# saugns/saugns

Measured on AMD Instinct MI355X. Metric: mono samples/sec/GPU @ N voices (depth-3 FM), higher is better.
Workload: dtype f32 (f64 table interpolation, u32 phase)

## Files before the change

### saugns_amd/csrc/hip_backend.hip

```cpp
#include <hip/hip_runtime.h>
#include "hip_backend.h"
#include "launch_plan.h"
#include "sau_dev_ops.h"
#include <stdio.h>
#include <stdlib.h>
#include <string.h>
#include <deque>
#include <map>
#include <memory>
#include <mutex>
#include <string>
#include <type_traits>
#include <vector>

namespace sauhip {

using namespace saudev;
using sauengine::BackendConfig;
using sauengine::tune_env;
using sauengine::SegmentDesc;
using namespace sauplan;

#include "k_common.h"
#include "k_block_loop.h"
// ... 127 lines not shown
		err = std::string(pinned ? "hipHostMalloc: " : "hipMalloc: ") + hipGetErrorString(e);
		return nullptr;
	}
	return q;
}
static void pool_free(bool pinned, void *q, size_t bytes) {
	if (!q) return;
	if (!BufPool::get().give(pinned, q, bytes)) { if (pinned) (void)hipHostFree(q); else (void)hipFree(q); }
}

static std::mutex &attr_mutex() { static std::mutex *m = new std::mutex; return *m; }
static bool raise_lds_attr(const void *fn, size_t lds, int dev, std::string &err) {
	static std::map<std::pair<const void *, int>, size_t> *slots = new std::map<std::pair<const void *, int>, size_t>;
	std::lock_guard<std::mutex> lk(attr_mutex());
	size_t &configured = (*slots)[std::make_pair(fn, dev & 15)];
	if (lds > configured) {
		hipError_t e = hipFuncSetAttribute(fn, hipFuncAttributeMaxDynamicSharedMemorySize, (int)lds);
		if (e != hipSuccess) { err = std::string("hipFuncSetAttribute: ") + hipGetErrorString(e); return false; }
		configured = lds;
	}
	return true;
}

enum : unsigned { FK_WIDE = 1, FK_TAIL = 2, FK_CUB = 4, FK_INNER = 8, FK_LANEMAJOR = 16 };
static const void *fast_kernel_fn(int build, uint32_t rows, unsigned form) {
	struct Entry { int build; uint32_t rows; unsigned form; const void *fn; };
#define FK(build, form, ...) {build, FK_ROWS(__VA_ARGS__), form, (const void *)fast_kernel<__VA_ARGS__>}
#define FK_ROWS(rows, ...) rows
	static const Entry table[] = {
		FK(0, 0, 2, 0), FK(0, 0, 4, 0), FK(0, 0, 5, 0), FK(0, 0, 6, 0), FK(0, 0, 8, 0),
		FK(1, 0, 2, 1), FK(1, 0, 4, 1),
		FK(2, 0, 2, 2), FK(2, 0, 4, 2), FK(2, 0, 5, 2), FK(2, 0, 6, 2), FK(2, 0, 8, 2),
		FK(3, 0, 4, 3), FK(3, 0, 5, 3), FK(3, 0, 6, 3),
		FK(0, FK_WIDE, 6, 0, false, true), FK(0, FK_WIDE, 8, 0, false, true), FK(0, FK_WIDE, 10, 0, false, true), FK(0, FK_WIDE, 12, 0, false, true),
		FK(2, FK_WIDE | FK_TAIL, 8, 2, false, true, true), FK(2, FK_WIDE, 8, 2, false, true), FK(2, FK_TAIL, 8, 2, false, false, true),
		FK(2, FK_CUB, (int)FAST_CUB_ROWS, 2, true),
		FK(0, FK_WIDE | FK_INNER | FK_LANEMAJOR, 12, 0, false, true, false, true, true), FK(0, FK_WIDE | FK_INNER, 12, 0, false, true, false, true),
		FK(0, FK_CUB, (int)FAST_CUB_ROWS, 0, true)};
#undef FK
#undef FK_ROWS
	for (const Entry &e : table)
		if (e.build == build && e.rows == rows && e.form == form) return e.fn;
	return nullptr;
}
static const void *repair_kernel_fn(uint32_t rows, bool wide) {
	if (wide)
		return rows == 12 ? (const void *)repair_kernel<12, true> : rows == 10 ? (const void *)repair_kernel<10, true>
		     : rows == 8 ? (const void *)repair_kernel<8, true> : rows == 6 ? (const void *)repair_kernel<6, true> : nullptr;
	return rows == 8 ? (const void *)repair_kernel<8> : rows == 6 ? (const void *)repair_kernel<6> : rows == 5 ? (const void *)repair_kernel<5>
	     : rows == 4 ? (const void *)repair_kernel<4> : rows == 2 ? (const void *)repair_kernel<2> : nullptr;
}
static const void *render_kernel_fn(uint32_t W, uint32_t T, uint32_t V, bool HB) {
	struct Entry { uint32_t W, T, V; bool HB; const void *fn; };
#define RK(W, T, V, HB) {W, T, V, HB, (const void *)render_kernel<W, T, V, HB>}
	static const Entry table[] = {
		RK(1, 4, 8, false), RK(1, 3, 8, false), RK(1, 2, 8, false), RK(1, 1, 8, false),
		RK(1, 4, 16, false), RK(1, 3, 16, false), RK(1, 2, 16, false), RK(1, 1, 16, false),
		RK(1, 1, 1, true), RK(1, 1, 1, false), RK(4, 4, 1, false), RK(8, 2, 1, false)};
#undef RK
	for (const Entry &e : table)
		if (e.W == W && e.T == T && e.V == V && e.HB == HB) return e.fn;
	return nullptr;
}

template <typename T, bool PINNED> struct PoolBuf {
	T *p = nullptr;
	size_t cap = 0, bytes = 0;
// ... 711 lines not shown
		}
		j.early_mixed_blocks = mixed_blocks;
		fp.range_mode = 0; fp.f_lo = 0; fp.f_hi = 0; fp.range_last = 0;
		return true;
	}

	bool launch_closed_form(Job &j, std::string &err) {
		const SegmentDesc &seg = j.seg;
		const FastPlan &k = j.fk;
		FastParams &fp = j.fp;
		fp.dyn_chunks = k.tasks.dyn_chunks; fp.dyn_static = k.tasks.dyn_static; fp.dyn_small = k.tasks.dyn_small;
		if (k.queues) {
			fp.inmix_flags = k.inmix_flags;
			fp.inmix_div_s = k.div.s; fp.inmix_div_m = k.div.m;
			if (k.inmix) {
				fp.inmix_stream = sets_[j.set].mstreams.p;
				fp.inmix_pcm_offset = seg.pcm_offset;
				hipLaunchKernelGGL(premix_kernel, dim3((seg.n_voices + 63) / 64), dim3(64), 0, stream_, fp);
				j.inmix_live = true;
			}
		}
		if (k.inner != INNER_NONE) {
			const bool lm = k.inner == INNER_LANE_MAJOR;
			const void *ik = fast_kernel_fn(0, 12, FK_WIDE | FK_INNER | (lm ? FK_LANEMAJOR : 0u));
			const size_t lds = k.inner_lds();
			FastParams ep = fp;
			ep.mode = 0; ep.edge_only = 1; ep.dyn_static = 1; ep.dyn_chunks = 2; ep.dyn_small = 0; ep.inmix_flags = 0;
			if (!launch_build(j, err, 0, k.rows, k.grid_edge, &ep, false, true)) j.launched = false;
			fp.mode = 0;
			void *iargs[] = {(void *)&fp};
			if (!raise_lds_attr(ik, lds, dev_, err)) return false;
			if (fp.inmix_flags && !pcm_hazard(err)) return false;
			HIP_OK(hipLaunchKernel(ik, dim3(k.grid), dim3(1024), iargs, lds, stream_));
			if (inner_report_) fprintf(stderr, "[sau-amd] inner: %s, %u voices\n", lm ? "lane-major" : "row-major", seg.n_voices);
		} else {
			if (inner_report_) fprintf(stderr, "[sau-amd] inner: none (rows %u, wide %d, chunks %u), %u voices\n", k.rows, k.wide_cf ? 1 : 0, fp.dyn_chunks, seg.n_voices);
			if (fp.inmix_flags && (!rows_hazard(j, err) || !pcm_hazard(err))) return false;
			launch_fast(j, err, 0);
		}
		fp.dyn_chunks = 0; fp.inmix_flags = 0; fp.dyn_small = 0;
		return true;
	}

	bool launch_cub(Job &j, std::string &err) {
		if (!j.fp.cub_ok) return true;
		const FastPlan &k = j.fk;
		FastParams q = k.main_build == 2 ? j.cfp : j.fp;
		q.n_fast = k.n_fast_cf; q.rows = FAST_CUB_ROWS; q.mode = 0; q.only_multi = 0;
		q.dyn_chunks = k.tasks_cub.dyn_chunks; q.dyn_static = k.tasks_cub.dyn_static;
		const size_t qlds = k.launch_lds(0, FAST_CUB_ROWS, false, true);
		const void *ck = fast_kernel_fn(0, FAST_CUB_ROWS, FK_CUB);
		if (!raise_lds_attr(ck, qlds, dev_, err)) return false;
		void *qargs[] = {(void *)&q};
		if (!rows_hazard(j, err)) return false;
		HIP_OK(hipLaunchKernel(ck, dim3(k.grid_cub), dim3(1024), qargs, qlds, stream_));
		return true;
	}
// ... 1393 lines not shown
```

### saugns_amd/csrc/k_fast_group_lm.h

```cpp
		const int j0 = l * T;
		const int t0 = (int)(cg * GF) - (int)H + j0;
		const uint32_t om = ((1u << T) - 1u) & ~((1u << min(max((int)H - j0, 0), T)) - 1u);
		auto prev32 = [&](const uint32_t *x, int k) -> uint32_t { return k > 0 ? x[k - 1] : lane_prev(x[T - 1]); };
		auto prev64 = [&](const double *x, int k) -> double { return k > 0 ? x[k - 1] : lane_prev(x[T - 1]); };
		const bool quads = ((cg * GF - H) & 3u) == 0;
		auto store_row = [&](float *row, const float *x, const bool nt) {
			uint32_t o = om;
			asm volatile("" : "+v"(o));
			if (quads) {
#pragma unroll
				for (int q = 0; q < T / 4; ++q) {
					const uint32_t oq = (o >> (4 * q)) & 15u;
					if (oq == 15u) {
						const fk_f32x4 v4 = {x[4 * q], x[4 * q + 1], x[4 * q + 2], x[4 * q + 3]};
						fk_f32x4 *p = (fk_f32x4 *)(row + t0 + 4 * q);
						if (nt) FK_VSTORE(p, v4); else *p = v4;
					} else if (oq != 0u) {
#pragma unroll
						for (int u = 0; u < 4; ++u)
							if ((oq >> u) & 1u) { if (nt) FK_VSTORE(&row[t0 + 4 * q + u], x[4 * q + u]); else row[t0 + 4 * q + u] = x[4 * q + u]; }
					}
				}
			} else {
#pragma unroll
// ... 32 lines not shown
					bool done = false;
					if (FK_COMMON && f.tab >= 0 && !has_fpm && !(f.ramp & 2)) {
						uint32_t ph[T];
						{
							uint32_t acc = f.phase0 + f.inc * (uint32_t)(t0 + 1);
#pragma unroll
							for (int k = 0; k < T; ++k) { ph[k] = acc; acc += f.inc; }
						}
						bool ok = true;
						if (has_pm) {
							float pm[T];
							bool big = false;
#pragma unroll
							for (int k = 0; k < T; ++k) {
								pm[k] = blk[k];
								big |= !(fabsf(pm[k]) < 0x1p20f);
							}
							ok = !__any(big);
#pragma unroll
							for (int k = 0; k < T; ++k) ph[k] += rint32w_p31_small(pm[k]);
						}
						if (ok) {
							const uint32_t ltab = tabs + (uint32_t)f.tab * FkTab<WIDE>::BYTES;
							double Is[T];
#pragma unroll
							for (int k = 0; k < T; ++k) Is[k] = fk_poly(fk_entry<WIDE>(ltab, ph[k]), ph[k]);
							if (FK_CONSTD && !has_pm && f.inc != 0) {
								const double x = (double)div_f32_normal(f.diff_scale, (float)(int32_t)f.inc);
#pragma unroll
								for (int k = 0; k < T; ++k)
									s[k] = (float)((Is[k] - prev64(Is, k)) * x + (double)f.diff_offset);
								done = true;
							} else {
								uint32_t dmin = 0xffffffffu;
#pragma unroll
								for (int k = 0; k < T; ++k) {
									uint32_t pp = prev32(ph, k);
									if (k == 0) asm("" : "+v"(pp));
									const int32_t d = (int32_t)(ph[k] - pp);
									dmin = min(dmin, (uint32_t)d);
									s[k] = wosc_diff(Is[k], prev64(Is, k), d, f.diff_scale, f.diff_offset);
								}
								done = true;
								if (__any(dmin == 0u)) {
									uint32_t hz = 0;
#pragma unroll
									for (int k = 0; k < T; ++k) hz |= ph[k] == prev32(ph, k) ? 1u << k : 0u;
									done = !__any((hz & dm) != 0u);
								}
							}
						}
					}
					if (!done) {
						uint32_t ph[T];
						double Is[T];
						float fv[T];
						{
							uint32_t acc = f.phase0 + f.inc * (uint32_t)(t0 + 1);
#pragma unroll
							for (int k = 0; k < T; ++k) { ph[k] = acc; acc += f.inc; fv[k] = f.fc; }
						}
						if (has_pm && !has_fpm) {
							float pm[T];
							bool big = false;
#pragma unroll
							for (int k = 0; k < T; ++k) {
								pm[k] = blk[k];
								big |= !(fabsf(pm[k]) < 0x1p20f);
							}
							if (!__any(big)) {
#pragma unroll
								for (int k = 0; k < T; ++k) ph[k] += rint32w_p31_small(pm[k]);
							} else {
#pragma unroll
								for (int k = 0; k < T; ++k) ph[k] += rint32w_p31(pm[k]);
							}
						} else if (has_fpm) {
#pragma unroll
							for (int k = 0; k < T; ++k) ph[k] += pm_offset32(false, true, 0.f, blk[k], fv[k]);
						}
						if (f.tab >= 0) {
							const uint32_t ltab = tabs + (uint32_t)f.tab * FkTab<WIDE>::BYTES;
#pragma unroll
							for (int k = 0; k < T; ++k) Is[k] = fk_poly(fk_entry<WIDE>(ltab, ph[k]), ph[k]);
						} else {
							const uint32_t wave = (f.type >> 8) & 0xff;
							const HerpC23 *g23 = P.g_c23 + (size_t)wave * WAVE_LEN;
							const HerpC01 *g01 = P.g_c01 + (size_t)wave * WAVE_LEN;
#pragma unroll
							for (int k = 0; k < T; ++k) {
								const uint32_t ind = ph[k] >> SLEN_BITS;
								Is[k] = herp_poly(g23[ind], g01[ind], ph[k]);
							}
						}
						uint32_t hz = 0;
						if (FK_CONSTD && !has_pm && !has_fpm && f.inc != 0) {
							const double x = (double)div_f32_normal(f.diff_scale, (float)(int32_t)f.inc);
#pragma unroll
							for (int k = 0; k < T; ++k) {
								const double pIs = prev64(Is, k);
								s[k] = (float)((Is[k] - pIs) * x + (double)f.diff_offset);
							}
						} else {
#pragma unroll
							for (int k = 0; k < T; ++k) {
								const uint32_t pph = prev32(ph, k);
								const double pIs = prev64(Is, k);
// ... 146 lines not shown
```

### saugns_amd/csrc/k_fast_voice.h

```cpp
#ifndef FK_TEMPORAL_ROWS
#define FK_VSTORE(p, v) __builtin_nontemporal_store((v), (p))
#else
#define FK_VSTORE(p, v) (*(p) = (v))
#endif
#ifndef FK_TEMPORAL_ROWS
#define FK_CSTORE(p, v) __builtin_nontemporal_store((v), (p))
#define FK_CLOAD(p) __builtin_nontemporal_load(p)
#else
#define FK_CSTORE(p, v) (*(p) = (v))
#define FK_CLOAD(p) (*(p))
#endif

__device__ __forceinline__ uint32_t lane_prev(uint32_t x) {
	return (uint32_t)__builtin_amdgcn_update_dpp(0, (int)x, 0x138 , 0xf, 0xf, true);
}
__device__ __forceinline__ double lane_prev(double x) {
	const uint32_t lo = lane_prev((uint32_t)__double2loint(x));
	const uint32_t hi = lane_prev((uint32_t)__double2hiint(x));
	return __hiloint2double((int)hi, (int)lo);
}

typedef double __attribute__((ext_vector_type(2))) fk_f64x2;
typedef float __attribute__((ext_vector_type(2))) fk_f32x2;
typedef float __attribute__((ext_vector_type(4))) fk_f32x4;
typedef const fk_f64x2 __attribute__((address_space(3))) *fk_lds_f64x2;
typedef const fk_f32x2 __attribute__((address_space(3))) *fk_lds_f32x2;
struct FkHerp { double c3, c2, c1, c0; };
template <bool WIDE, bool TAB0 = false>
__device__ __forceinline__ FkHerp fk_entry(const uint32_t tab, const uint32_t ph) {
	FkHerp h;
	if (WIDE && TAB0) {
		const uint32_t a = (ph >> (SLEN_BITS - 4)) & ((WAVE_LEN - 1) << 4);
		const fk_f64x2 hi = *(fk_lds_f64x2)(uintptr_t)a;
		const fk_f64x2 lo = *(fk_lds_f64x2)(uintptr_t)(a + FkTab<true>::C01);
		h.c3 = hi.x; h.c2 = hi.y; h.c1 = lo.x; h.c0 = lo.y;
	} else if (WIDE) {
		uint32_t ind = ph >> SLEN_BITS;
		asm("" : "+v"(ind));
		const uint32_t a = tab + (ind << 4);
		const fk_f64x2 hi = *(fk_lds_f64x2)(uintptr_t)a;
		const fk_f64x2 lo = *(fk_lds_f64x2)(uintptr_t)(a + FkTab<true>::C01);
		h.c3 = hi.x; h.c2 = hi.y; h.c1 = lo.x; h.c0 = lo.y;
	} else {
		const uint32_t ind = ph >> SLEN_BITS;
		const fk_f64x2 hi = *(fk_lds_f64x2)(uintptr_t)(tab + ind * 16u);
		const fk_f32x2 lo = *(fk_lds_f32x2)(uintptr_t)(tab + FkTab<false>::C01 + ind * 8u);
		h.c3 = hi.x; h.c2 = hi.y; h.c1 = (double)lo.x; h.c0 = (double)lo.y;
	}
	return h;
}
__device__ __forceinline__ double fk_poly(const FkHerp &h, const uint32_t ph) {
	const double x = (double)(ph & (SLEN - 1));
	return ((h.c3 * x + h.c2) * x + h.c1) * x + h.c0;
}
__device__ __forceinline__ double fk_poly_rise(const FkHerp &h, const uint32_t ph) {
	const double x = (double)(ph & (SLEN - 1));
	return ((h.c3 * x + h.c2) * x + h.c1) * x;
}
template <bool WIDE>
__device__ __forceinline__ void fk_stage_tables(const FastParams &P, unsigned char *lds, const uint32_t tid, const uint32_t nthreads) {
	for (uint32_t t = 0; t < P.n_tabs; ++t) {
		const uint32_t wave = P.wave_of_tab[t];
		const uint4 *s23 = (const uint4 *)(P.g_c23 + (size_t)wave * WAVE_LEN);
		uint4 *d23 = (uint4 *)(lds + (size_t)t * FkTab<WIDE>::BYTES);
		for (uint32_t i = tid; i < WAVE_LEN; i += nthreads) d23[i] = s23[i];
		const HerpC01 *s01 = P.g_c01 + (size_t)wave * WAVE_LEN;
		if (WIDE) {
			fk_f64x2 *d01 = (fk_f64x2 *)(lds + (size_t)t * FkTab<WIDE>::BYTES + FkTab<WIDE>::C01);
			for (uint32_t i = tid; i < WAVE_LEN; i += nthreads) { fk_f64x2 v; v.x = (double)s01[i].c1; v.y = (double)s01[i].c0; d01[i] = v; }
		} else {
			uint2 *d01 = (uint2 *)(lds + (size_t)t * FkTab<WIDE>::BYTES + FkTab<WIDE>::C01);
			for (uint32_t i = tid; i < WAVE_LEN; i += nthreads) d01[i] = ((const uint2 *)s01)[i];
		}
	}
}

__device__ __forceinline__ FastStep load_step_uniform(const FastStep *p) {
	const_u32_ptr q = (const_u32_ptr)(uintptr_t)p;
	union { FastStep s; uint32_t u[20]; } c;
#pragma unroll
	for (int i = 0; i < 20; ++i) c.u[i] = q[i];
	return c.s;
}

template <int T, int SCAN, bool REPAIR = false, bool CUB = false, bool WIDE = false, int SPLIT = 0 , bool TAIL = false>
__device__ __forceinline__ void fast_voice(const FastParams &P, const uint32_t v, const FastInfo &fi,
		float *slots, unsigned long long *carry, const uint32_t tabs , const int l,
		const uint32_t wpv, const uint32_t cstart, unsigned long long *lring = nullptr,
		const uint32_t dyn_c = 0, const uint32_t dyn_k = 0 ,
		const uint32_t vpos = ~0u ,
		const uint32_t wg_waves = 16u ) {
	constexpr int NP = 64 * T;
	(void)NP;
	const uint32_t fast_total = uni(fi.total);
	if (fast_total == 0) return;
	if ((uni(fi.cub) != 0) != CUB) return;
	const VoiceDesc vd = P.voices[v];
	const uint32_t H = uni(fi.H);

	constexpr bool FULL = SCAN == 1;
	constexpr bool CH = SCAN == 1 || SCAN == 3;
	const uint32_t li = CH ? fast_list_of(P.mode, P.sum_levels) : 0u;
	const uint32_t n_fsteps = uni(li == 0 ? fi.n_fsteps : li == 1 ? fi.n_pass[0] : li == 2 ? fi.n_pass[1] : li == 3 ? fi.n_pass[2] : fi.n_pass[3]);
	const size_t list_at = ((size_t)li * P.n_voices + v) * P.max_steps;
	const FastStep *fsteps = P.fsteps + list_at;
	const FastLine *flines = P.flines + list_at;
	const FastAux *faux = P.faux + list_at;
	const FastLine *fplines = P.fplines ? P.fplines + list_at : nullptr;
// ... 33 lines not shown
			} else {
				it_lo = P.f_lo / tc;
				n_iter = fast_total <= P.f_hi ? ngroups : min(ngroups, P.f_hi / tc);
				if (P.f_lo >= fast_total) n_iter = 0;
			}
		}
	}
	if (!REPAIR && SCAN == 0 && dyn_k) {
		(void)fk_chunk_groups(ngroups, dyn_k, P.dyn_small, dyn_c, it_lo, n_iter);
	}
	if constexpr (!REPAIR && SCAN == 0 && WIDE && T == 12 && SPLIT == 0) {
		if (P.edge_only) {
			if (dyn_c && last_group == 0) return;
			it_lo = dyn_c ? last_group : 0u;
			n_iter = it_lo + 1;
		}
	}
	const uint32_t tail_n = (TAIL && SCAN == 2 && !REPAIR && !CUB && P.tail_ok) ? uni(fi.tail) : 0u;
	const uint32_t tail_s = tail_n ? uni(fi.tail_stream) : 0u;
	(void)tail_s;
	uint32_t cgm = cstart;
#define FKG_ADVANCE() (it += gstride, cgm = cgm + wpv >= lk_ring ? cgm + wpv - lk_ring : cgm + wpv)
	if constexpr (SPLIT == 3 && SCAN == 0 && !REPAIR && !CUB && !TAIL) {
		for (uint32_t it = it_lo + cstart; it < n_iter; FKG_ADVANCE()) {
			if (it == 0 || it == last_group) continue;
			const uint32_t cg = it;
#include "k_fast_group_lm.h"
		}
	} else if constexpr (SPLIT == 2 && !REPAIR) {
		for (uint32_t it = it_lo + cstart; it < n_iter; FKG_ADVANCE()) {
			if (it == 0 || it == last_group) continue;
			const uint32_t cg = it, repair_rows = 0;
			constexpr bool EDGE = false;
#include "k_fast_group.h"
		}
	} else if constexpr (SPLIT == 1 && !REPAIR) {
		uint32_t it = it_lo + cstart;
		if (it < n_iter && (it == 0 || it == last_group)) {
			const uint32_t cg = it, repair_rows = 0;
			constexpr bool EDGE = true;
#include "k_fast_group.h"
			FKG_ADVANCE();
		}
		for (; it < n_iter && it != last_group; FKG_ADVANCE()) {
			const uint32_t cg = it, repair_rows = 0;
			constexpr bool EDGE = false;
#include "k_fast_group.h"
// ... 175 lines not shown
	uint32_t j = vi + A.nvc - first;
	if (j >= A.nvc) j -= A.nvc;
	if (kc < 8 || j >= tpc) return;
	if (inmix_ctl(A, INMIX_CHUNK + INMIX_LINE * (kc - 8) + INMIX_DONE) != A.nvc) return;
	__builtin_amdgcn_fence(__ATOMIC_ACQUIRE, "agent");
	if (A.flags & 4u) return;
	for (; j < tpc; j += A.nvc) {
		inmix_tile(A, cs, ce, j, l);
		if (l == 0) __hip_atomic_fetch_or(&A.ctl[INMIX_CHUNK + INMIX_LINE * (kc - 8) + INMIX_BITS + (j >> 5)], 1u << (j & 31u), __ATOMIC_RELAXED, __HIP_MEMORY_SCOPE_AGENT);
	}
}

#ifndef FK_SPLIT_MASK
#define FK_SPLIT_MASK 9
#endif
#ifndef FK_MINB
#define FK_MINB 1
#endif
#ifdef FK_WAVES_EU
#define FK_ATTR __launch_bounds__(1024) __attribute__((amdgpu_waves_per_eu(FK_WAVES_EU)))
#else
#define FK_ATTR __launch_bounds__(1024, FK_MINB)
#endif
template <int T, int SCAN, bool CUB = false, bool WIDE = false, bool TAIL = false, bool INNER = false, bool LM = false>
__global__ void FK_ATTR fast_kernel(FastParams P) {
	static_assert(!INNER || (SCAN == 0 && WIDE && T == 12 && !CUB && !TAIL), "the inner-groups-only form exists for the 12-row wide closed-form build");
	static_assert(!LM || INNER, "the lane-major form exists for the inner-groups-only build");
	static_assert(!WIDE || ((SCAN == 0 || SCAN == 2) && !CUB), "only the closed-form and the look-back builds have a wide-table form");
	static_assert(!TAIL || (SCAN == 2 && !CUB && T == 8), "the stream-mixing form exists for the 8-row look-back build");
	constexpr int NP = 64 * T;
	constexpr int W = 16;
	constexpr int SPLIT = INNER ? (LM ? 3 : 2) : (!CUB && ((SCAN == 0 && T == 8 && (FK_SPLIT_MASK & 1)) || (SCAN == 0 && T == 10 && (FK_SPLIT_MASK & 2)) ||
	                                (SCAN == 0 && T == 12 && (FK_SPLIT_MASK & 4)) || (SCAN == 2 && T == 8 && (FK_SPLIT_MASK & 8)))) ? 1 : 0;
	extern __shared__ __align__(16) unsigned char lds[];
	const int tid = threadIdx.x;
	const int w = (int)uni((uint32_t)tid >> 6);
	const int l = tid & 63;
	if (SCAN == 1 && P.mode != 0 && P.mode <= P.sum_levels && P.pass_flags[P.mode - 1] == 0) return;
	if (SCAN == 1 && P.mode == P.sum_levels + 2 && P.pass_flags[FAST_MAX_LEVELS + 1] == 0) return;
	if (SCAN == 1 && P.only_multi && P.pass_flags[FAST_MAX_LEVELS + 2] == 0) return;
	if (SCAN == 3 && P.pass_flags[FAST_LEAN_FLAG] == 0) return;
	if (SCAN == 0 && P.split_cf && P.pass_flags[FAST_CF_COUNT] == 0) return;
	if (CUB && P.pass_flags[FAST_CUB_FLAG] == 0) return;
	if (SCAN == 2 && P.pass_flags[FAST_LK_COUNT] == 0) return;

	const uint32_t tabs = (uint32_t)(uintptr_t)lds;
	unsigned char *areas = lds + (size_t)P.n_tabs * FkTab<WIDE>::BYTES;
	const size_t area_bytes = (size_t)P.n_fast * NP * sizeof(float) + (size_t)P.max_steps * sizeof(unsigned long long);
// ... 12 lines not shown
	const uint32_t NV = P.n_voices;
	if (SCAN == 0) {
		const uint32_t NVc = P.split_cf ? P.pass_flags[FAST_CF_COUNT] : NV;
		const uint32_t K = P.dyn_chunks ? P.dyn_chunks : 1u, n_tasks = NVc * K;
		const bool counted = P.dyn_static == 0;
		const uint32_t stride = gridDim.x * W;
		uint32_t snext = blockIdx.x * W + (uint32_t)w;
		const bool im = !CUB && (P.inmix_flags & 64u) != 0;
		const bool mixing = im && (P.inmix_flags & 32u) && uni(__hip_atomic_load(&P.work_count[1], __ATOMIC_RELAXED, __HIP_MEMORY_SCOPE_AGENT)) == 0;
		for (;;) {
			uint32_t t_ = snext;
			if (counted && !im) { t_ = 0; if (l == 0) t_ = atomicAdd(&P.pass_flags[FAST_DYN_CTR], 1u); }
			if (!CUB && im) {
				const InmixArgs A = inmix_args(NVc);
				const unsigned long long nx = inmix_next(A, mixing ? A.ctl[INMIX_NCH] : K, l);
				t_ = nx == ~0ull ? n_tasks : (uint32_t)nx * K + (uint32_t)(nx >> 32);
			}
			const uint32_t task = uni(t_);
			if (task >= n_tasks) break;
			snext = task + stride;
			const uint32_t vi = task / K;
			const uint32_t v = P.split_cf ? P.vlists[vi] : vi;
			const FastInfo fi = P.info[v];
			fast_voice<T, 0, false, CUB, WIDE, SPLIT>(P, v, fi, slots, carry, tabs, l, 1u, 0u, nullptr, task - vi * K, K);
			if (!CUB && mixing) {
				const InmixArgs A = inmix_args(NVc);
				inmix_after(A, task - vi * K, vi, l);
			}
		}
		return;
	}
	const uint32_t g = blockIdx.x * W + (uint32_t)w;
	const uint32_t total_waves = gridDim.x * W;
	if (SCAN == 2) {
		const uint32_t NVl = P.pass_flags[FAST_LK_COUNT];
		uint32_t wpv = P.look_wpv;
		if (P.look_words_real) {
			wpv = total_waves / NVl;
			if (wpv > P.look_groups) wpv = P.look_groups;
			wpv = wpv >= 64 ? 64u : wpv >= 32 ? 32u : wpv >= 16 ? 16u : wpv >= 8 ? 8u : wpv >= 4 ? 4u : wpv >= 2 ? 2u : 1u;
		}
		const uint32_t slots_v = total_waves / wpv;
		const bool spread = wpv >= 32 && (P.look_wpv_flags & 4u);
		const uint32_t j0 = spread ? g % slots_v : g / wpv, cs = spread ? g / slots_v : g % wpv;
		if (j0 >= slots_v || cs >= wpv) return;
		for (uint32_t j = j0; j < NVl; j += slots_v) {
			const uint32_t v = P.vlists[NV + j];
// ... 127 lines not shown
```

### saugns_amd/csrc/launch_plan.h

```cpp
#ifndef SAU_LAUNCH_PLAN_H
#define SAU_LAUNCH_PLAN_H

#include "engine.h"
#include "mix_overlap.h"
#include "sau_dev_math.h"
#include <string.h>

namespace sauplan {

using namespace saudev;
using sauengine::SegmentDesc;

#ifndef FK_GRID
#define FK_GRID 256
#endif
constexpr uint32_t FAST_TAB_BYTES = (uint32_t)(WAVE_LEN * (sizeof(HerpC23) + sizeof(HerpC01))), FAST_TAB_BYTES_WIDE = 65536u;
constexpr uint32_t FAST_MAX_SCAN = 8;
constexpr uint32_t LOOK_LDS_BYTES = FAST_MAX_SCAN * 2 * 64 * sizeof(unsigned long long);
constexpr uint32_t FAST_MAX_LEVELS = 3;
constexpr uint32_t FAST_CUB_ROWS = 4;
constexpr uint32_t FAST_LISTS = 5;
constexpr uint32_t INMIX_NSMALL = 8;
#ifndef SAU_CHAIN_BATCH_FRAMES
#define SAU_CHAIN_BATCH_FRAMES 32
// ... 25 lines not shown
	bool wide_look = true;
	uint32_t more_rows = 12;
	bool repair = true;
	bool analyze_lds = true;
	bool chain = true;
	bool chain_inline = true;
	bool chain_early = true;
	uint32_t chain_chunks = 0;
	uint32_t chain_chunk_frames = 16384;
	bool short_last_chunk = true;
	bool chain_alone = false;
	bool lean = true;
	uint32_t lean_rows = 6;
	bool dyn = true;
	uint32_t dyn_groups = 12;
	uint32_t dyn_floor = 24;
	uint32_t dyn_min_tasks = 2;
	bool xcd_queues = true;
	bool inmix = true;
	uint32_t inmix_min_voices = 64;
	uint32_t inmix_min_steps = 2;
	bool inmix_taper = false;
	uint32_t inmix_at = 13;
	bool inmix_dry = false;
	bool inner = true;
	bool lanemajor = true;
	bool duo = true;
	uint32_t duo_lw = 0, duo_prio = 0;
	bool tailmix = false;
	bool mix_few = true;
	bool early_mix = true;
	bool mix64 = true;
	bool poison = false;
	bool mix_overlap = true;
	bool mix_overlap_shared = false;
	uint32_t mix_overlap_mb = 4096;
	bool mix_overlap_fail = false;
};

inline Tuning tuning_from_env(const char *(*env)(const char *)) {
	Tuning t;
	auto off = [&](const char *name) { return env(name) == nullptr; };
	auto num = [&](const char *name, uint32_t &v) { if (const char *s = env(name)) v = (uint32_t)atoi(s); };
	auto at_least_1 = [&](const char *name, uint32_t &v) { if (const char *s = env(name)) { const int n = atoi(s); v = n >= 1 ? (uint32_t)n : 1u; } };
	const char *wt = env("SAU_AMD_GEOMETRY");
	t.geo = (wt && !strcmp(wt, "8x2")) ? 0 : 1;
// ... 21 lines not shown
	t.repair = off("SAU_AMD_NO_REPAIR");
	t.analyze_lds = off("SAU_AMD_ANALYZE_NO_LDS");
	t.chain = off("SAU_AMD_NO_CHAIN");
	t.chain_inline = off("SAU_AMD_NO_CHAIN_INLINE");
	t.chain_early = off("SAU_AMD_NO_EARLY_CHAINS");
	if (const char *cc = env("SAU_AMD_CHAIN_CHUNKS")) {
		const int n = atoi(cc);
		t.chain_chunks = n >= 32 ? 32 : n >= 1 ? (uint32_t)n : 1;
	}
	if (const char *cf = env("SAU_AMD_CHAIN_CHUNK_FRAMES")) { const int n = atoi(cf); if (n >= 4096) t.chain_chunk_frames = (uint32_t)n; }
	t.short_last_chunk = off("SAU_AMD_NO_SHORT_LAST_CHUNK");
	if (const char *ca = env("SAU_AMD_CHAIN_ALONE")) t.chain_alone = atoi(ca) != 0;
	t.lean = off("SAU_AMD_NO_LEAN");
	num("SAU_AMD_LEAN_ROWS", t.lean_rows);
	t.dyn = off("SAU_AMD_NO_DYN");
	at_least_1("SAU_AMD_DYN_GROUPS", t.dyn_groups);
	at_least_1("SAU_AMD_DYN_FLOOR", t.dyn_floor);
	at_least_1("SAU_AMD_DYN_MIN_TASKS", t.dyn_min_tasks);
	t.xcd_queues = off("SAU_AMD_NO_XCD_QUEUES");
	t.inmix = off("SAU_AMD_NO_INMIX");
	num("SAU_AMD_INMIX_MIN_VOICES", t.inmix_min_voices);
	num("SAU_AMD_INMIX_MIN_STEPS", t.inmix_min_steps);
	t.inmix_taper = !off("SAU_AMD_INMIX_TAPER");
	if (const char *ia = env("SAU_AMD_INMIX_AT")) t.inmix_at = (uint32_t)atoi(ia) & 15u;
	t.inmix_dry = !off("SAU_AMD_INMIX_DRY");
	t.inner = off("SAU_AMD_NO_INNER");
	t.lanemajor = off("SAU_AMD_NO_LANEMAJOR");
	t.duo = off("SAU_AMD_NO_DUO");
	if (const char *lw = env("SAU_AMD_DUO_LW")) t.duo_lw = (uint32_t)atoi(lw) & 15u;
	if (const char *pr = env("SAU_AMD_DUO_PRIO")) t.duo_prio = (uint32_t)atoi(pr) & 7u;
	t.tailmix = !off("SAU_AMD_TAILMIX");
	t.mix_few = off("SAU_AMD_NO_MIX_FEW");
	t.early_mix = off("SAU_AMD_NO_EARLY_MIX");
	t.mix64 = off("SAU_AMD_NO_MIX64");
	t.poison = !off("SAU_AMD_POISON");
	t.mix_overlap = off("SAU_AMD_NO_MIX_OVERLAP");
	t.mix_overlap_shared = !off("SAU_AMD_MIX_OVERLAP_SHARED");
	if (const char *mb = env("SAU_AMD_MIX_OVERLAP_MB")) { const long n = atol(mb); t.mix_overlap_mb = n < 0 ? 0u : n > 0x7fffffffl ? 0x7fffffffu : (uint32_t)n; }
	t.mix_overlap_fail = !off("SAU_AMD_MIX_OVERLAP_FAIL");
	return t;
}

struct DeviceLimits {
	size_t lds_limit = 160 * 1024;
	uint32_t fk_grid = FK_GRID;
	uint32_t cus = 256;
	bool eight_xcds = true;
// ... 145 lines not shown
	}
	return q;
}
inline Tasks static_tasks(const SegmentDesc &seg, uint32_t n_groups, uint32_t grid) {
	Tasks q;
	uint32_t k = grid * 16 / seg.n_voices;
	if (k > n_groups) k = n_groups;
	q.dyn_chunks = k ? k : 1; q.dyn_static = 1;
	return q;
}
struct MagicDiv { uint32_t m = 0, s = 0; };
inline MagicDiv magic_div(uint32_t d) {
	MagicDiv q;
	while ((1ull << q.s) < d) ++q.s;
	q.m = (uint32_t)(((1ull << (32 + q.s)) / d) + 1ull - (1ull << 32));
	return q;
}
inline uint32_t magic_quotient(uint32_t q, MagicDiv d) {
	if (d.s == 0) return q;
	const uint32_t t = (uint32_t)(((unsigned long long)q * d.m) >> 32);
	return (t + ((q - t) >> 1)) >> (d.s - 1);
}

enum Inner : uint32_t { INNER_NONE = 0, INNER_ROW_MAJOR = 1, INNER_LANE_MAJOR = 2 };
enum Mixer : uint32_t { MIX_NONE = 0, MIX_FEW_F32, MIX_F32, MIX_FEW, MIX_64, MIX_256 };

struct FastPlan {
	bool use_fast = false;
	bool seq_ok = false;
	bool look_split = false;
	int main_build = 0;
	uint32_t fmax_steps = 0, n_fast = 0, n_fast_cf = 0;
	uint32_t rows = 2;
	uint32_t rows_multi = 2;
	uint32_t rows_cf = 2;
	uint32_t rows_lean = 4;
	bool lean_on = false;
	TableMap tabs;
	uint32_t n_want = 0;
	bool wide_cf = false;
	bool wide_look = false;
	bool cub_ok = false;
	uint32_t sum_levels = 2;
	uint32_t scan_groups = 0;
	bool scan = false;
	bool look = false;
	size_t look_words = 0;
	bool look_words_real = false;
	uint32_t look_wpv = 1;
	bool look_inside = true;
	uint32_t look_wpv_flags = 0;
	bool inc_rows = false;
	uint32_t inc_stride = 0;
	bool chains = false;
	uint32_t chain_stride = 0, chain_grid = 0;
	TableMap ctabs;
	ChainChunks chunks;
	uint32_t pass_grid = 0;
	bool early_mix = false;
	bool split_cf = false, duo = false, tailmix = false;
	bool queues = false;
	bool inmix = false;
	uint32_t inmix_flags = 0;
	MagicDiv div;
	Inner inner = INNER_NONE;
	Tasks tasks, tasks_cf, tasks_cub;
	uint32_t groups = 0, groups_cf = 0;
	uint32_t grid = 1, grid_cf = 1, grid_look = 1, grid_edge = 1, grid_cub = 1, grid_repair = 1;
	uint32_t rows_repair = 2;

	void drop_chains() { chains = false; lean_on = false; }
	size_t launch_lds(int build, uint32_t r, bool wide, bool cf = false) const {
		return tabs.n * (size_t)(wide ? FAST_TAB_BYTES_WIDE : FAST_TAB_BYTES) + 16 * buf_area(cf ? n_fast_cf : n_fast, r, fmax_steps) +
			(build == 2 ? LOOK_LDS_BYTES : 0);
	}
	size_t inner_lds() const {
		return inner == INNER_LANE_MAJOR ? tabs.n * (size_t)FAST_TAB_BYTES_WIDE : launch_lds(0, rows, true);
	}
};

inline void plan_rows(FastPlan &p, const SegmentDesc &seg, const Tuning &tun, const DeviceLimits &dev) {
	p.fmax_steps = seg.max_steps < 64 ? seg.max_steps : 64;
	uint32_t FT = tun.fast_rows;
	p.look_split = tun.seq && seg.may_scan && tun.two_pass && tun.lookback && tun.look_rows != 0 && seg.n_voices >= tun.look_min_voices;
	if (tun.seq && seg.may_scan && FT > 4 && !p.look_split) FT = 4;
	if (p.look_split && FT > tun.look_rows) FT = rows_at_most(tun.look_rows);
	p.seq_ok = tun.seq && seg.may_scan;
	p.n_fast = p.seq_ok && seg.n_fast_full > seg.n_fast ? seg.n_fast_full : seg.n_fast;
// ... 95 lines not shown
}

inline void plan_closed_form(FastPlan &p, const SegmentDesc &seg, const Tuning &tun, const DeviceLimits &dev, const PlanInputs &in) {
	if (p.main_build == 0) p.tasks = plan_tasks(seg, tun, p.groups, p.grid);
	p.queues = tun.xcd_queues && dev.eight_xcds && p.main_build == 0 && !p.tasks.dyn_static && p.tasks.dyn_chunks >= 16 && !p.cub_ok;
	if (p.queues) {
		p.inmix_flags = 64u;
		if (tun.inmix_taper) {
			const uint32_t G = task_groups(seg, tun);
			const uint32_t small = G / 4 ? G / 4 : 1;
			if (p.groups >= 32 * G + INMIX_NSMALL * small) {
				p.tasks.dyn_small = small;
				p.tasks.dyn_chunks = (p.groups - INMIX_NSMALL * small + G - 1) / G + INMIX_NSMALL;
			}
		}
		p.div = magic_div(seg.n_voices);
		p.inmix = tun.inmix && !in.f32 && seg.n_streams == 1 && in.max_write && seg.n_voices >= tun.inmix_min_voices &&
			seg.max_steps >= tun.inmix_min_steps && in.row_stride < (1u << 24);
		if (p.inmix)
			p.inmix_flags = 64u | 32u | (seg.stereo ? 1u : 0u) | (seg.swap_bytes ? 2u : 0u) | (tun.inmix_dry ? 4u : 0u) | ((tun.inmix_at & 15u) << 8);
	}
	if (tun.inner && p.main_build == 0 && p.wide_cf && p.rows == 12 && p.tasks.dyn_chunks >= 3)
		p.inner = tun.lanemajor && p.n_fast == 1 ? INNER_LANE_MAJOR : INNER_ROW_MAJOR;
	p.grid_edge = wave_grid(2ull * seg.n_voices, dev.fk_grid);
}

inline FastPlan plan_fast(const SegmentDesc &seg, const Tuning &tun, const DeviceLimits &dev, const PlanInputs &in) {
	FastPlan p;
	plan_rows(p, seg, tun, dev);
	plan_sums(p, seg, tun, dev);
	p.groups = row_groups(seg.len, p.rows);
	p.grid = group_grid(seg.n_voices, p.groups, dev.fk_grid);
	plan_chains(p, seg, tun, dev, in);
	if (p.use_fast && p.main_build == 2) plan_split(p, seg, tun, dev, in);
	if (p.use_fast && !p.scan) plan_closed_form(p, seg, tun, dev, in);
	const uint32_t g4 = row_groups(seg.len, FAST_CUB_ROWS);
	p.grid_cub = group_grid(seg.n_voices, g4, dev.fk_grid);
	p.tasks_cub = static_tasks(seg, g4, p.grid_cub);
	p.rows_repair = p.main_build == 2 ? p.rows_cf : p.rows;
	p.grid_repair = wave_grid(seg.n_voices, 64);
	return p;
}

inline Mixer plan_mixer(const SegmentDesc &seg, const Tuning &tun, const PlanInputs &in, size_t pcm_pitch, bool inmix_live,
		uint32_t early_blocks) {
	if (!in.max_write) return MIX_NONE;
// ... 267 lines not shown
```

Measured before the change: 250.7 million.

## Software-pipeline LDS table reads and fuse phase/diff pass in lane-major inner kernel

Restructures the lane-major inner group loop so that Hermite table entries are fetched one pair of samples ahead through volatile-ordered LDS reads, with scheduling barriers that overlap each load with the polynomial evaluation of the previous pair. It also folds the per-sample integral and difference computation into a single pass with a paired reciprocal-based division, which avoids keeping a full array of double integrals live. A separate lane-major in-mix trigger point is added, and an optional single-table kernel variant is added but compiled out by default. The fences are meant to limit register pressure and hide LDS latency, at the cost of a more rigid instruction schedule.

```diff
diff --git a/saugns_amd/csrc/hip_backend.hip b/saugns_amd/csrc/hip_backend.hip
--- a/saugns_amd/csrc/hip_backend.hip
+++ b/saugns_amd/csrc/hip_backend.hip
@@ -173,7 +173,7 @@
 	return true;
 }
 
-enum : unsigned { FK_WIDE = 1, FK_TAIL = 2, FK_CUB = 4, FK_INNER = 8, FK_LANEMAJOR = 16 };
+enum : unsigned { FK_WIDE = 1, FK_TAIL = 2, FK_CUB = 4, FK_INNER = 8, FK_LANEMAJOR = 16, FK_TAB0 = 32 };
 static const void *fast_kernel_fn(int build, uint32_t rows, unsigned form) {
 	struct Entry { int build; uint32_t rows; unsigned form; const void *fn; };
 #define FK(build, form, ...) {build, FK_ROWS(__VA_ARGS__), form, (const void *)fast_kernel<__VA_ARGS__>}
@@ -187,6 +187,9 @@
 		FK(2, FK_WIDE | FK_TAIL, 8, 2, false, true, true), FK(2, FK_WIDE, 8, 2, false, true), FK(2, FK_TAIL, 8, 2, false, false, true),
 		FK(2, FK_CUB, (int)FAST_CUB_ROWS, 2, true),
 		FK(0, FK_WIDE | FK_INNER | FK_LANEMAJOR, 12, 0, false, true, false, true, true), FK(0, FK_WIDE | FK_INNER, 12, 0, false, true, false, true),
+#if FK_LM_TAB0
+		FK(0, FK_WIDE | FK_INNER | FK_LANEMAJOR | FK_TAB0, 12, 0, false, true, false, true, true, true),
+#endif
 		FK(0, FK_CUB, (int)FAST_CUB_ROWS, 0, true)};
 #undef FK
 #undef FK_ROWS
@@ -194,6 +197,12 @@
 		if (e.build == build && e.rows == rows && e.form == form) return e.fn;
 	return nullptr;
 }
+#if FK_LM_TAB0
+static bool tab0_kernel_ok(const void *fn) {
+	static const bool ok = [&] { hipFuncAttributes a; return fn && hipFuncGetAttributes(&a, fn) == hipSuccess && a.sharedSizeBytes == 0; }();
+	return ok;
+}
+#endif
 static const void *repair_kernel_fn(uint32_t rows, bool wide) {
 	if (wide)
 		return rows == 12 ? (const void *)repair_kernel<12, true> : rows == 10 ? (const void *)repair_kernel<10, true>
@@ -951,7 +960,13 @@
 		}
 		if (k.inner != INNER_NONE) {
 			const bool lm = k.inner == INNER_LANE_MAJOR;
-			const void *ik = fast_kernel_fn(0, 12, FK_WIDE | FK_INNER | (lm ? FK_LANEMAJOR : 0u));
+#if FK_LM_TAB0
+			const bool tab0 = lm && k.inner_tab0 && tab0_kernel_ok(fast_kernel_fn(0, 12, FK_WIDE | FK_INNER | FK_LANEMAJOR | FK_TAB0));
+#else
+			const bool tab0 = false;
+#endif
+			const void *ik = fast_kernel_fn(0, 12, FK_WIDE | FK_INNER | (lm ? FK_LANEMAJOR : 0u) | (tab0 ? FK_TAB0 : 0u));
+			if (!ik) { err = "no inner instantiation of fast_kernel for this form"; return false; }
 			const size_t lds = k.inner_lds();
 			FastParams ep = fp;
 			ep.mode = 0; ep.edge_only = 1; ep.dyn_static = 1; ep.dyn_chunks = 2; ep.dyn_small = 0; ep.inmix_flags = 0;
@@ -961,7 +976,7 @@
 			if (!raise_lds_attr(ik, lds, dev_, err)) return false;
 			if (fp.inmix_flags && !pcm_hazard(err)) return false;
 			HIP_OK(hipLaunchKernel(ik, dim3(k.grid), dim3(1024), iargs, lds, stream_));
-			if (inner_report_) fprintf(stderr, "[sau-amd] inner: %s, %u voices\n", lm ? "lane-major" : "row-major", seg.n_voices);
+			if (inner_report_) fprintf(stderr, "[sau-amd] inner: %s, %u voices, %u tables%s\n", lm ? "lane-major" : "row-major", seg.n_voices, k.tabs.n, tab0 ? ", tab0" : "");
 		} else {
 			if (inner_report_) fprintf(stderr, "[sau-amd] inner: none (rows %u, wide %d, chunks %u), %u voices\n", k.rows, k.wide_cf ? 1 : 0, fp.dyn_chunks, seg.n_voices);
 			if (fp.inmix_flags && (!rows_hazard(j, err) || !pcm_hazard(err))) return false;
diff --git a/saugns_amd/csrc/k_fast_group_lm.h b/saugns_amd/csrc/k_fast_group_lm.h
--- a/saugns_amd/csrc/k_fast_group_lm.h
+++ b/saugns_amd/csrc/k_fast_group_lm.h
@@ -78,9 +78,75 @@
 						}
 						if (ok) {
 							const uint32_t ltab = tabs + (uint32_t)f.tab * FkTab<WIDE>::BYTES;
+							static_assert(T % 2 == 0, "pairs of samples");
+							auto hermite = [&](auto &&sink) {
+#if FK_LM_AHEAD > 0
+								constexpr int NP2 = T / 2, A = FK_LM_AHEAD < NP2 ? FK_LM_AHEAD : NP2 - 1, NS = A + 1;
+								FkHerp q[2 * NS];
+#pragma unroll
+								for (int p = 0; p < A; ++p) {
+									q[2 * p] = fk_entry<WIDE, TAB0, true>(ltab, ph[2 * p]);
+									q[2 * p + 1] = fk_entry<WIDE, TAB0, true>(ltab, ph[2 * p + 1]);
+								}
+#pragma unroll
+								for (int p = 0; p < NP2; ++p) {
+									if (p + A < NP2) {
+										const int sl = (p + A) % NS;
+										q[2 * sl] = fk_entry<WIDE, TAB0, true>(ltab, ph[2 * (p + A)]);
+										q[2 * sl + 1] = fk_entry<WIDE, TAB0, true>(ltab, ph[2 * (p + A) + 1]);
+									}
+									__builtin_amdgcn_sched_barrier(0);
+									const int sl = p % NS;
+									sink(2 * p, fk_poly(q[2 * sl], ph[2 * p]), fk_poly(q[2 * sl + 1], ph[2 * p + 1]));
+								}
+#define FK_LM_PIN(...) asm volatile("" : __VA_ARGS__)
+#else
+#pragma unroll
+								for (int k = 0; k < T; k += 2)
+									sink(k, fk_poly(fk_entry<WIDE, TAB0>(ltab, ph[k]), ph[k]), fk_poly(fk_entry<WIDE, TAB0>(ltab, ph[k + 1]), ph[k + 1]));
+#define FK_LM_PIN(...) ((void)0)
+#endif
+							};
+#if FK_LM_ONE_PHASE_SET
+							double I0 = 0., Ip = 0.;
+							if (FK_CONSTD && !has_pm && f.inc != 0) {
+								const double x = (double)div_f32_normal(f.diff_scale, (float)(int32_t)f.inc);
+								hermite([&](const int k, const double Ia, const double Ib) {
+									if (k == 0) I0 = Ia;
+									else s[k] = (float)((Ia - Ip) * x + (double)f.diff_offset);
+									s[k + 1] = (float)((Ib - Ia) * x + (double)f.diff_offset);
+									Ip = Ib;
+									if (k == 0) FK_LM_PIN("+v"(I0), "+v"(s[1]));
+									else FK_LM_PIN("+v"(s[k]), "+v"(s[k + 1]));
+								});
+								s[0] = (float)((I0 - lane_prev(Ip)) * x + (double)f.diff_offset);
+								done = true;
+							} else {
+								uint32_t dmin = 0xffffffffu;
+								uint32_t pp = lane_prev(ph[T - 1]);
+								asm("" : "+v"(pp));
+								const int32_t d0 = (int32_t)(ph[0] - pp);
+#pragma unroll
+								for (int k = 0; k < T; ++k) asm volatile("" : "+v"(ph[k]));
+								double x0 = 0.;
+								hermite([&](const int k, const double Ia, const double Ib) {
+									const int32_t da = k == 0 ? d0 : (int32_t)(ph[k] - ph[k - 1]), db = (int32_t)(ph[k + 1] - ph[k]);
+									dmin = min(dmin, min((uint32_t)da, (uint32_t)db));
+									const fk_f32x2 dv = {(float)da, (float)db};
+									const fk_f32x2 x = fk_div_diff_scale2(f.diff_scale, dv);
+									if (k == 0) { I0 = Ia; x0 = (double)x.x; }
+									else s[k] = (float)((Ia - Ip) * (double)x.x + (double)f.diff_offset);
+									s[k + 1] = (float)((Ib - Ia) * (double)x.y + (double)f.diff_offset);
+									Ip = Ib;
+									if (k == 0) FK_LM_PIN("+v"(I0), "+v"(x0), "+v"(s[1]), "+v"(dmin));
+									else FK_LM_PIN("+v"(s[k]), "+v"(s[k + 1]), "+v"(dmin));
+								});
+								s[0] = (float)((I0 - lane_prev(Ip)) * x0 + (double)f.diff_offset);
+								done = !__any(dmin == 0u);
+							}
+#else
 							double Is[T];
-#pragma unroll
-							for (int k = 0; k < T; ++k) Is[k] = fk_poly(fk_entry<WIDE>(ltab, ph[k]), ph[k]);
+							hermite([&](const int k, const double Ia, const double Ib) { Is[k] = Ia; Is[k + 1] = Ib; FK_LM_PIN("+v"(Is[k]), "+v"(Is[k + 1])); });
 							if (FK_CONSTD && !has_pm && f.inc != 0) {
 								const double x = (double)div_f32_normal(f.diff_scale, (float)(int32_t)f.inc);
 #pragma unroll
@@ -105,6 +171,8 @@
 									done = !__any((hz & dm) != 0u);
 								}
 							}
+#endif
+#undef FK_LM_PIN
 						}
 					}
 					if (!done) {
@@ -112,9 +180,13 @@
 						double Is[T];
 						float fv[T];
 						{
-							uint32_t acc = f.phase0 + f.inc * (uint32_t)(t0 + 1);
-#pragma unroll
-							for (int k = 0; k < T; ++k) { ph[k] = acc; acc += f.inc; fv[k] = f.fc; }
+							uint32_t inc = f.inc;
+#if FK_LM_ONE_PHASE_SET
+							asm volatile("" : "+s"(inc));
+#endif
+							uint32_t acc = f.phase0 + inc * (uint32_t)(t0 + 1);
+#pragma unroll
+							for (int k = 0; k < T; ++k) { ph[k] = acc; acc += inc; fv[k] = f.fc; }
 						}
 						if (has_pm && !has_fpm) {
 							float pm[T];
@@ -138,7 +210,7 @@
 						if (f.tab >= 0) {
 							const uint32_t ltab = tabs + (uint32_t)f.tab * FkTab<WIDE>::BYTES;
 #pragma unroll
-							for (int k = 0; k < T; ++k) Is[k] = fk_poly(fk_entry<WIDE>(ltab, ph[k]), ph[k]);
+							for (int k = 0; k < T; ++k) Is[k] = fk_poly(fk_entry<WIDE, TAB0>(ltab, ph[k]), ph[k]);
 						} else {
 							const uint32_t wave = (f.type >> 8) & 0xff;
 							const HerpC23 *g23 = P.g_c23 + (size_t)wave * WAVE_LEN;
diff --git a/saugns_amd/csrc/k_fast_voice.h b/saugns_amd/csrc/k_fast_voice.h
--- a/saugns_amd/csrc/k_fast_voice.h
+++ b/saugns_amd/csrc/k_fast_voice.h
@@ -11,6 +11,10 @@
 #define FK_CLOAD(p) (*(p))
 #endif
 
+#if FK_LM_ONE_PHASE_SET && !FK_LM_AHEAD
+#error "FK_LM_ONE_PHASE_SET needs FK_LM_AHEAD: without its fences the compiler's schedule of the one loop spills (216 VGPRs)"
+#endif
+
 __device__ __forceinline__ uint32_t lane_prev(uint32_t x) {
 	return (uint32_t)__builtin_amdgcn_update_dpp(0, (int)x, 0x138 , 0xf, 0xf, true);
 }
@@ -26,10 +30,23 @@
 typedef const fk_f64x2 __attribute__((address_space(3))) *fk_lds_f64x2;
 typedef const fk_f32x2 __attribute__((address_space(3))) *fk_lds_f32x2;
 struct FkHerp { double c3, c2, c1, c0; };
-template <bool WIDE, bool TAB0 = false>
+typedef const volatile fk_f64x2 __attribute__((address_space(3))) *fk_lds_f64x2_ord;
+template <bool WIDE, bool TAB0 = false, bool ORDERED = false>
 __device__ __forceinline__ FkHerp fk_entry(const uint32_t tab, const uint32_t ph) {
 	FkHerp h;
-	if (WIDE && TAB0) {
+	static_assert(!ORDERED || WIDE, "the ordered reads exist for the wide table block");
+	if (WIDE && ORDERED) {
+		uint32_t a;
+		if (TAB0) a = (ph >> (SLEN_BITS - 4)) & ((WAVE_LEN - 1) << 4);
+		else {
+			uint32_t ind = ph >> SLEN_BITS;
+			asm("" : "+v"(ind));
+			a = tab + (ind << 4);
+		}
+		const fk_f64x2 hi = *(fk_lds_f64x2_ord)(uintptr_t)a;
+		const fk_f64x2 lo = *(fk_lds_f64x2_ord)(uintptr_t)(a + FkTab<true>::C01);
+		h.c3 = hi.x; h.c2 = hi.y; h.c1 = lo.x; h.c0 = lo.y;
+	} else if (WIDE && TAB0) {
 		const uint32_t a = (ph >> (SLEN_BITS - 4)) & ((WAVE_LEN - 1) << 4);
 		const fk_f64x2 hi = *(fk_lds_f64x2)(uintptr_t)a;
 		const fk_f64x2 lo = *(fk_lds_f64x2)(uintptr_t)(a + FkTab<true>::C01);
@@ -57,6 +74,13 @@
 	const double x = (double)(ph & (SLEN - 1));
 	return ((h.c3 * x + h.c2) * x + h.c1) * x;
 }
+__device__ __forceinline__ fk_f32x2 fk_div_diff_scale2(const float a, const fk_f32x2 b) {
+	fk_f32x2 r;
+	r.x = __builtin_amdgcn_rcpf(b.x); r.y = __builtin_amdgcn_rcpf(b.y);
+	const fk_f32x2 av = {a, a};
+	const fk_f32x2 q = av * r;
+	return __builtin_elementwise_fma(__builtin_elementwise_fma(-b, q, av), r, q);
+}
 template <bool WIDE>
 __device__ __forceinline__ void fk_stage_tables(const FastParams &P, unsigned char *lds, const uint32_t tid, const uint32_t nthreads) {
 	for (uint32_t t = 0; t < P.n_tabs; ++t) {
@@ -83,7 +107,8 @@
 	return c.s;
 }
 
-template <int T, int SCAN, bool REPAIR = false, bool CUB = false, bool WIDE = false, int SPLIT = 0 , bool TAIL = false>
+template <int T, int SCAN, bool REPAIR = false, bool CUB = false, bool WIDE = false, int SPLIT = 0 , bool TAIL = false,
+		bool TAB0 = false >
 __device__ __forceinline__ void fast_voice(const FastParams &P, const uint32_t v, const FastInfo &fi,
 		float *slots, unsigned long long *carry, const uint32_t tabs , const int l,
 		const uint32_t wpv, const uint32_t cstart, unsigned long long *lring = nullptr,
@@ -163,7 +188,8 @@
 	uint32_t cgm = cstart;
 #define FKG_ADVANCE() (it += gstride, cgm = cgm + wpv >= lk_ring ? cgm + wpv - lk_ring : cgm + wpv)
 	if constexpr (SPLIT == 3 && SCAN == 0 && !REPAIR && !CUB && !TAIL) {
-		for (uint32_t it = it_lo + cstart; it < n_iter; FKG_ADVANCE()) {
+		if (TAB0 && tabs != 0u) zero_acc = 1;
+		else for (uint32_t it = it_lo + cstart; it < n_iter; FKG_ADVANCE()) {
 			if (it == 0 || it == last_group) continue;
 			const uint32_t cg = it;
 #include "k_fast_group_lm.h"
@@ -385,8 +411,9 @@
 #else
 #define FK_ATTR __launch_bounds__(1024, FK_MINB)
 #endif
-template <int T, int SCAN, bool CUB = false, bool WIDE = false, bool TAIL = false, bool INNER = false, bool LM = false>
+template <int T, int SCAN, bool CUB = false, bool WIDE = false, bool TAIL = false, bool INNER = false, bool LM = false, bool TAB0 = false>
 __global__ void FK_ATTR fast_kernel(FastParams P) {
+	static_assert(!TAB0 || LM, "the one-table address form exists for the lane-major inner build");
 	static_assert(!INNER || (SCAN == 0 && WIDE && T == 12 && !CUB && !TAIL), "the inner-groups-only form exists for the 12-row wide closed-form build");
 	static_assert(!LM || INNER, "the lane-major form exists for the inner-groups-only build");
 	static_assert(!WIDE || ((SCAN == 0 || SCAN == 2) && !CUB), "only the closed-form and the look-back builds have a wide-table form");
@@ -445,7 +472,7 @@
 			const uint32_t vi = task / K;
 			const uint32_t v = P.split_cf ? P.vlists[vi] : vi;
 			const FastInfo fi = P.info[v];
-			fast_voice<T, 0, false, CUB, WIDE, SPLIT>(P, v, fi, slots, carry, tabs, l, 1u, 0u, nullptr, task - vi * K, K);
+			fast_voice<T, 0, false, CUB, WIDE, SPLIT, false, TAB0>(P, v, fi, slots, carry, tabs, l, 1u, 0u, nullptr, task - vi * K, K);
 			if (!CUB && mixing) {
 				const InmixArgs A = inmix_args(NVc);
 				inmix_after(A, task - vi * K, vi, l);
diff --git a/saugns_amd/csrc/launch_plan.h b/saugns_amd/csrc/launch_plan.h
--- a/saugns_amd/csrc/launch_plan.h
+++ b/saugns_amd/csrc/launch_plan.h
@@ -71,6 +71,7 @@
 	uint32_t inmix_min_steps = 2;
 	bool inmix_taper = false;
 	uint32_t inmix_at = 13;
+	uint32_t inmix_at_lm = 15;
 	bool inmix_dry = false;
 	bool inner = true;
 	bool lanemajor = true;
@@ -138,7 +139,7 @@
 	num("SAU_AMD_INMIX_MIN_VOICES", t.inmix_min_voices);
 	num("SAU_AMD_INMIX_MIN_STEPS", t.inmix_min_steps);
 	t.inmix_taper = !off("SAU_AMD_INMIX_TAPER");
-	if (const char *ia = env("SAU_AMD_INMIX_AT")) t.inmix_at = (uint32_t)atoi(ia) & 15u;
+	if (const char *ia = env("SAU_AMD_INMIX_AT")) t.inmix_at = t.inmix_at_lm = (uint32_t)atoi(ia) & 15u;
 	t.inmix_dry = !off("SAU_AMD_INMIX_DRY");
 	t.inner = off("SAU_AMD_NO_INNER");
 	t.lanemajor = off("SAU_AMD_NO_LANEMAJOR");
@@ -330,6 +331,16 @@
 	return (t + ((q - t) >> 1)) >> (d.s - 1);
 }
 
+#ifndef FK_LM_ONE_PHASE_SET
+#define FK_LM_ONE_PHASE_SET 1
+#endif
+#ifndef FK_LM_TAB0
+#define FK_LM_TAB0 0
+#endif
+#ifndef FK_LM_AHEAD
+#define FK_LM_AHEAD 1
+#endif
+constexpr bool FK_LM_SHORT_TASKS = FK_LM_ONE_PHASE_SET && FK_LM_AHEAD;
 enum Inner : uint32_t { INNER_NONE = 0, INNER_ROW_MAJOR = 1, INNER_LANE_MAJOR = 2 };
 enum Mixer : uint32_t { MIX_NONE = 0, MIX_FEW_F32, MIX_F32, MIX_FEW, MIX_64, MIX_256 };
 
@@ -372,6 +383,7 @@
 	uint32_t inmix_flags = 0;
 	MagicDiv div;
 	Inner inner = INNER_NONE;
+	bool inner_tab0 = false;
 	Tasks tasks, tasks_cf, tasks_cub;
 	uint32_t groups = 0, groups_cf = 0;
 	uint32_t grid = 1, grid_cf = 1, grid_look = 1, grid_edge = 1, grid_cub = 1, grid_repair = 1;
@@ -513,6 +525,8 @@
 	}
 	if (tun.inner && p.main_build == 0 && p.wide_cf && p.rows == 12 && p.tasks.dyn_chunks >= 3)
 		p.inner = tun.lanemajor && p.n_fast == 1 ? INNER_LANE_MAJOR : INNER_ROW_MAJOR;
+	p.inner_tab0 = p.inner == INNER_LANE_MAJOR && p.tabs.n == 1;
+	if (FK_LM_SHORT_TASKS && p.inmix && p.inner == INNER_LANE_MAJOR) p.inmix_flags = (p.inmix_flags & ~(15u << 8)) | ((tun.inmix_at_lm & 15u) << 8);
 	p.grid_edge = wave_grid(2ull * seg.n_voices, dev.fk_grid);
 }
 
```

After: 254.0 million (median of 6 runs). 1.3% higher.
